# shwetabhardwaj44/EfficientVideoClassification_Youtube8M

Measured on AMD Instinct MI355X. Metric: frames/sec (whole node) H-LSTM teacher+student B=256x300x1152; GAP@20, higher is better.
Workload: dtype bf16; 1 GPU; HierarchicalLstmModel teacher_student every_n=10, lstm_cells=1024x2, MoE(2), batch 256 x 300 x 1152 per GPU; global_batch=256, frames_per_video=300, parallelism=dp1, num_frames=U{120..300}

## Files before the change

### efficientvideoclassification_youtube8m_amd/_lib.py

```python
from __future__ import annotations

import ctypes as C
import os

_HERE = os.path.dirname(os.path.abspath(__file__))
LIB_PATH = os.environ.get("EVC_LIB", os.path.join(_HERE, "libevc_hip.so"))

vp, i32, i64, f32 = C.c_void_p, C.c_int, C.c_int64, C.c_float

SIGNATURES = {
    "evc_check_device": [i32],
    "evc_l2norm_chunk_fwd": [vp, vp, vp, i32, i32, i32, i32, vp, i32, i32, vp, i32, vp, vp, i32, vp, i32, vp, i32, vp],
    "evc_sort_rows_by_len": [vp, i32, i32, vp, vp, vp, vp],
    "evc_frame_counts": [vp, i32, i32, i32, i32, i32, i32, vp, vp, vp, vp],
    "evc_gemm_nt": [vp, i64, vp, i64, vp, i64, i32, i32, i32, vp, i32, i32, vp],
    "evc_gemm_nt_sqnorm": [vp, i64, vp, i64, vp, i64, i32, i32, i32, vp, f32, vp, vp, i64, vp],
    "evc_gemm_tn": [vp, i64, vp, i64, vp, i64, i32, i32, i32, i32, i32, vp],
    "evc_gemm_tn2": [vp, i64, vp, i64, i32, vp, i64, i32, i32, vp, i64, i32, i32, i32, i32, vp],
    "evc_gemm_tn2_rows": [vp, i64, vp, i64, i32, vp, i64, i32, i32, vp, i64, i32, i32, i32, vp, i32, i32, vp],
    "evc_gemm_tn2_slabs": [vp, i64, vp, i64, i32, vp, i64, i32, i32, vp, i64, i64, i32, i32, i32, i32, vp],
    "evc_sum_slabs": [vp, i64, i32, i32, i32, i64, vp, i64, i32, vp],
    "evc_colsum_bf16": [vp, i64, i32, i32, i32, vp, vp],
    "evc_colsum_bf16_det": [vp, i64, i32, i32, i32, vp, vp, i32, vp],
    "evc_lstm_layer_fwd": [vp, vp, vp, vp, i32, i32, i32, i32, i32, vp, vp, vp, vp, i64, vp, vp, vp, vp, vp],
    "evc_lstm_layer_fwd_hp": [vp, vp, i64, vp, i64, vp, vp, i32, i32, i32, i32, vp, vp, vp, vp, vp, i64, vp, vp, vp],
    "evc_gemm_nt_split": [vp, i64, vp, i64, vp, i64, i32, i32, i32, vp, vp],
    "evc_cast_f32_to_f16_wide": [vp, i64, i32, i32, i32, i32, i32, vp, vp],
    "evc_cast_f32_to_bf16_wide": [vp, i64, i32, i32, vp, i64, i32, vp],
    "evc_lstm_layer_fwd_f16": [vp, i64, vp, vp, vp, i32, i32, i32, i32, vp, i32, vp, vp, vp, i64, vp, vp, vp, vp, vp],
    "evc_lstm_layer_fwd_f16_fp8lo": [vp, i64, i32, i64, i32, vp, vp, i32, i32, vp, vp, i32, i32, i32, vp, vp, vp, vp, i64, vp, vp, vp, vp, vp, vp, i32, vp],
    "evc_l2norm_chunk_int": [vp, vp, i32, i32, i32, i32, vp, i32, i32, vp, vp, vp, vp, vp, vp, i32, vp, i32, vp],
    "evc_lstm_level2_fwd_high": [vp, i64, i32, i64, i32, vp, vp, i32, i32, vp, vp, vp, i32, vp, i64, vp, vp, i32, i32, i32, vp, vp, vp, vp, vp, vp, vp, vp, i64,
                                 vp, vp, vp, vp, vp, vp, vp],
    "evc_lstm_layer_fwd_f16_dith": [vp, i64, i32, i64, i32, vp, i64, vp, i64, i32, vp, vp, i32, i32, i32, vp, vp, vp, vp, i64, vp, vp, vp, vp, vp],
    "evc_cast_f32_to_f16_dither": [vp, i64, i32, i64, C.c_uint32, vp, i64, i64, vp],
    "evc_lstm_stack2_fwd_f16_fp8lo": [vp, i32, vp, vp, vp, vp, vp, i32, i32, vp, vp, i32, i32, i32, i32, vp, vp, vp, vp, vp, vp, vp, vp, vp, i64, vp, vp, vp, vp, vp],
    "evc_cast_f32_to_fp8_lo": [vp, i64, i32, i32, i32, i32, i32, vp, i64, vp],
    "evc_cast_f32_to_fp8_lohi": [vp, i64, i32, i32, i32, i32, i32, vp, i64, vp],
    "evc_lstm_layer_bwd": [vp, vp, i32, i32, i32, i32, vp, vp, vp, vp, i64, vp, vp, vp, vp, vp, vp, vp, vp, vp],
    "evc_transpose_to_bf16": [vp, i32, i64, i32, i32, vp, i64, i32, i32, vp],
    "evc_cast_f32_to_bf16": [vp, i64, i32, i32, vp, i64, vp],
    "evc_cast_f32_to_f16": [vp, i64, i32, i32, vp, i64, vp],
    "evc_cast_f32_to_bf16_split": [vp, i64, i32, i32, vp, vp, i64, vp],
# ... 116 lines not shown
```

### efficientvideoclassification_youtube8m_amd/csrc/evc_gemm_tn.hip

```cpp
#include "gemm_shared.h"

struct StoreParamsT {
  float* C; long ldc; int M, N;
  int row_il_H;
  int accumulate, splits, ksteps_per_split;
  long slab_stride;
};

template <class Cfg, bool SEG = false>
__global__ __launch_bounds__(Cfg::NT) void gemm_tn_kernel(GemmOperandsT p, StoreParamsT s, int tiles_m, int tiles_n) {
  const int nwg = tiles_m * tiles_n;
  int bid = blockIdx.x, split = 0;
  if (s.splits > 1) {
    split = bid / nwg;
    bid -= split * nwg;
  }
  const int id = xcd_remap(bid, nwg);
  int tm, tn;
  tile_of(id, tiles_m, tiles_n, tm, tn, s.splits > 1 ? patch_rows(nwg, tiles_n) : 8);
  const int m0 = tm * Cfg::BM;
  int n0 = tn * Cfg::BU;
  int nb = n0;
  if (p.B2) {
    if (n0 >= p.N1) {
      p.B = p.B2; p.ldb = p.ldb2; nb = n0 - p.N1; p.N = s.N - p.N1;
      s.N = p.c_col2 + p.N;
      n0 = p.c_col2 + nb;
    } else {
      p.N = s.N = p.N1;
    }
  }
  if (SEG) {
    int off = split * s.ksteps_per_split, sg = 0;
    p.nk = min(s.ksteps_per_split, p.nk - off);
#pragma unroll
    for (int i = 0; i < 15; ++i) {
      const bool adv = sg == i && i + 1 < p.nseg && off >= (int)p.seg_len[i];
      off -= adv ? (int)p.seg_len[i] : 0;
      sg += adv ? 1 : 0;
    }
    p.seg0 = sg; p.seg_off0 = off;
  } else if (s.splits > 1) {
    const int k0 = split * s.ksteps_per_split;
    p.A += (long)k0 * 32 * p.lda;
    p.B += (long)k0 * 32 * p.ldb;
    p.nk = min(s.ksteps_per_split, p.nk - k0);
  }
  f32x4 acc[Cfg::MI][1][Cfg::NI];
  gemm_mainloop_tn<Cfg, true, TN_LOOP_MODE, SEG>(p, m0, nb, lds_dyn, acc);
  float* C = s.C + split * s.slab_stride;
  const int wave = threadIdx.x >> 6, wc = wave % Cfg::WC;
  const bool plain = s.slab_stride > 0 || (s.splits == 1 && !s.accumulate);
  const bool aligned = (s.ldc % 4) == 0 && ((uintptr_t)C % 16) == 0 && n0 + wc * Cfg::WU + Cfg::WU <= s.N;
  __syncthreads();
  if (plain && aligned) {
    store_tile_via_lds<Cfg, 4, false>(acc, lds_dyn, C, s.ldc, s.M, s.N, m0, n0, nullptr, s.row_il_H);
  } else if (s.splits == 1 && s.accumulate && aligned) {
    store_tile_via_lds<Cfg, 4, false, true>(acc, lds_dyn, C, s.ldc, s.M, s.N, m0, n0, nullptr, s.row_il_H);
  } else if (plain) {
    TileCoordsT<Cfg> tc;
#pragma unroll
    for (int mi = 0; mi < Cfg::MI; ++mi) {
      const int m = m0 + tc.row0 + mi * 16;
      if (m >= s.M) continue;
      const long mo = s.row_il_H > 0 ? (long)(m & 3) * s.row_il_H + (m >> 2) : m;
#pragma unroll
      for (int ni = 0; ni < Cfg::NI; ++ni)
#pragma unroll
        for (int r = 0; r < 4; ++r) {
          const int n = n0 + tc.unit0 + ni * 16 + r;
          if (n < s.N) C[mo * s.ldc + n] = acc[mi][0][ni][r];
        }
    }
  } else {
    store_tile_via_lds<Cfg, 4, true>(acc, lds_dyn, C, s.ldc, s.M, s.N, m0, n0, nullptr, s.row_il_H);
  }
}

static int gemm_tn_impl(const evc_bf16* A, int64_t lda, const evc_bf16* B, int64_t ldb, int N1, const evc_bf16* B2, int64_t ldb2,
                        int c_col2, float* C, int64_t ldc, int M, int N, int K, int row_interleave_H, int accumulate, void* stream,
                        int slab_rows = 0, const int32_t* rows_per_slab = nullptr) {
  EVC_REQUIRE(M >= 8 && N >= 8 && K > 0 && M % 8 == 0 && N % 8 == 0 && K % 32 == 0, EVC_ERR_BAD_SHAPE,
              "evc_gemm_tn: needs M %% 8 == 0, N %% 8 == 0, K %% 32 == 0 (M=%d N=%d K=%d)", M, N, K);
  EVC_REQUIRE(lda % 8 == 0 && ldb % 8 == 0 && ((uintptr_t)A % 16) == 0 && ((uintptr_t)B % 16) == 0, EVC_ERR_BAD_ALIGN,
              "evc_gemm_tn: operands must be 16-byte aligned (lda=%ld ldb=%ld)", (long)lda, (long)ldb);
  EVC_REQUIRE(row_interleave_H == 0 || M == 4 * row_interleave_H, EVC_ERR_BAD_SHAPE, "evc_gemm_tn: row_interleave_H needs M == 4*H");
  EVC_REQUIRE(!B2 || (N1 > 0 && N1 < N && N1 % 256 == 0 && ldb2 % 8 == 0 && ((uintptr_t)B2 % 16) == 0 && c_col2 >= N1), EVC_ERR_BAD_SHAPE,
              "evc_gemm_tn2: N1=%d must be a multiple of 256 inside (0, N=%d), B2 16-byte aligned with ldb2 %% 8 == 0, c_col2=%d >= N1", N1, N, c_col2);
  hipStream_t st = (hipStream_t)stream;
  GemmOperandsT p{A, lda, B, ldb, M, N, K / 32};
  if (B2) { p.B2 = B2; p.ldb2 = ldb2; p.N1 = N1; p.c_col2 = c_col2; }
  bool seg = false;
  if (rows_per_slab && slab_rows > 0 && slab_rows % 32 == 0 && K % slab_rows == 0 && !evc_deterministic()) {
    const int nslabs = K / slab_rows, slab_steps = slab_rows / 32;
    int n = 0, total = 0;
    const long ld_max = lda > ldb ? (long)lda : (long)ldb;
    bool ok = (long)nslabs * slab_steps < 65536 && (long)K * (B2 && ldb2 > ld_max ? (long)ldb2 : ld_max) * 2 < (1L << 32);
    for (int t = 0; t < nslabs && ok; ++t) {
      int r = rows_per_slab[t] < 0 ? 0 : (rows_per_slab[t] > slab_rows ? slab_rows : rows_per_slab[t]);
      const int steps = (r + 31) / 32;
      if (steps == 0) continue;
      if (n == 16) { ok = false; break; }
      p.seg_start[n] = (unsigned short)(t * slab_steps); p.seg_len[n] = (unsigned short)steps;
      ++n; total += steps;
    }
    if (ok && total > 0 && total < K / 32) { seg = true; p.nseg = n; p.nk = total; K = total * 32; }
  }
  typedef TileCfg2<128, 1, 128, 2, 4, 5, true> CfgTn128;
  if (forced_tile() == 11 || (forced_tile() == 0 && K <= 2048 && (long)ceil_div(M, 128) * ceil_div(N, 128) >= 192)) {
    const int tm1 = ceil_div(M, 128), tn1 = ceil_div(N, 128);
    StoreParamsT s1{C, ldc, M, N, row_interleave_H, accumulate, 1, p.nk, 0};
    if (seg) launch_cfg<CfgTn128>(gemm_tn_kernel<CfgTn128, true>, tm1 * tn1, st, p, s1, tm1, tn1);
    else launch_cfg<CfgTn128>(gemm_tn_kernel<CfgTn128>, tm1 * tn1, st, p, s1, tm1, tn1);
    EVC_LAUNCH_CHECK();
    return EVC_OK;
  }
  if (forced_tile() == 0 && N <= 128 && !B2) {
    const int tm1 = ceil_div(M, 128);
    int splits = 256 / tm1;
    if (splits > K / 1024) splits = K / 1024;
    if (splits < 1 || evc_deterministic()) splits = 1;
    while (splits > 1 && (long)ceil_div(p.nk, splits) * (splits - 1) >= p.nk) --splits;
    StoreParamsT s1{C, ldc, M, N, row_interleave_H, accumulate, splits, ceil_div(p.nk, splits), 0};
    if (splits > 1 && !accumulate) EVC_CHECK_HIP(hipMemset2DAsync(C, ldc * sizeof(float), 0, (size_t)N * sizeof(float), M, st));
    if (seg) launch_cfg<CfgTn128>(gemm_tn_kernel<CfgTn128, true>, tm1 * splits, st, p, s1, tm1, 1);
    else launch_cfg<CfgTn128>(gemm_tn_kernel<CfgTn128>, tm1 * splits, st, p, s1, tm1, 1);
    EVC_LAUNCH_CHECK();
    return EVC_OK;
  }
  const int tm = ceil_div(M, CfgPlainV2::BM), tn = ceil_div(N, CfgPlainV2::BU);
  int splits = 256 / (tm * tn);
  if (splits > K / 1024) splits = K / 1024;
  if (splits < 1 || evc_deterministic()) splits = 1;
  StoreParamsT s{C, ldc, M, N, row_interleave_H, accumulate, splits, ceil_div(p.nk, splits), 0};
  if (splits > 1 && !accumulate) EVC_CHECK_HIP(hipMemset2DAsync(C, ldc * sizeof(float), 0, (size_t)N * sizeof(float), M, st));
  if (seg) launch_cfg<CfgPlainV2>(gemm_tn_kernel<CfgPlainV2, true>, tm * tn * splits, st, p, s, tm, tn);
  else launch_cfg<CfgPlainV2>(gemm_tn_kernel<CfgPlainV2>, tm * tn * splits, st, p, s, tm, tn);
  EVC_LAUNCH_CHECK();
  return EVC_OK;
}

extern "C" int evc_gemm_tn2_rows(const evc_bf16* A, int64_t lda, const evc_bf16* B1, int64_t ldb1, int N1, const evc_bf16* B2, int64_t ldb2,
                                 int N2, int c_col2, float* C, int64_t ldc, int M, int slab_rows, int nslabs, const int32_t* rows_per_slab,
                                 int row_interleave_H, int accumulate, void* stream) {
  EVC_REQUIRE(B1 && N1 > 0 && slab_rows > 0 && nslabs > 0 && rows_per_slab && (long)slab_rows * nslabs < (1L << 31), EVC_ERR_BAD_ARG,
              "evc_gemm_tn2_rows: B1, N1, slab_rows, nslabs, rows_per_slab are required");
  EVC_REQUIRE(!B2 || N2 > 0, EVC_ERR_BAD_ARG, "evc_gemm_tn2_rows: N2=%d", N2);
  EVC_REQUIRE(!B2 || accumulate || c_col2 == N1, EVC_ERR_BAD_ARG, "evc_gemm_tn2_rows: segments that are not adjacent in C (c_col2=%d, N1=%d) need accumulate", c_col2, N1);
  return gemm_tn_impl(A, lda, B1, ldb1, B2 ? N1 : 0, B2, ldb2, B2 ? c_col2 : 0, C, ldc, M, N1 + (B2 ? N2 : 0), slab_rows * nslabs, row_interleave_H, accumulate,
                      stream, slab_rows, rows_per_slab);
}

extern "C" int evc_gemm_tn(const evc_bf16* A, int64_t lda, const evc_bf16* B, int64_t ldb, float* C, int64_t ldc,
                           int M, int N, int K, int row_interleave_H, int accumulate, void* stream) {
  return gemm_tn_impl(A, lda, B, ldb, 0, nullptr, 0, 0, C, ldc, M, N, K, row_interleave_H, accumulate, stream);
}

extern "C" int evc_gemm_tn2(const evc_bf16* A, int64_t lda, const evc_bf16* B1, int64_t ldb1, int N1, const evc_bf16* B2, int64_t ldb2,
                            int N2, int c_col2, float* C, int64_t ldc, int M, int K, int row_interleave_H, int accumulate, void* stream) {
  EVC_REQUIRE(B1 && B2 && N1 > 0 && N2 > 0, EVC_ERR_BAD_ARG, "evc_gemm_tn2: two column segments are required");
  EVC_REQUIRE(accumulate || c_col2 == N1, EVC_ERR_BAD_ARG, "evc_gemm_tn2: segments that are not adjacent in C (c_col2=%d, N1=%d) need accumulate "
              "(the split-K join adds into a C the caller has zeroed)", c_col2, N1);
  return gemm_tn_impl(A, lda, B1, ldb1, N1, B2, ldb2, c_col2, C, ldc, M, N1 + N2, K, row_interleave_H, accumulate, stream);
}

extern "C" int evc_gemm_tn_slabs(const evc_bf16* A, int64_t lda, const evc_bf16* B, int64_t ldb, float* slabs, int M, int N, int K,
                                 int nslab, void* stream) {
  EVC_REQUIRE(M >= 8 && N >= 8 && K > 0 && M % 8 == 0 && N % 8 == 0 && K % 32 == 0 && nslab >= 1 && nslab <= K / 32, EVC_ERR_BAD_SHAPE,
              "evc_gemm_tn_slabs: needs M %% 8 == 0, N %% 8 == 0, K %% 32 == 0, 1 <= nslab <= K/32 (M=%d N=%d K=%d nslab=%d)", M, N, K, nslab);
  EVC_REQUIRE(lda % 8 == 0 && ldb % 8 == 0 && ((uintptr_t)A % 16) == 0 && ((uintptr_t)B % 16) == 0, EVC_ERR_BAD_ALIGN,
              "evc_gemm_tn_slabs: operands must be 16-byte aligned (lda=%ld ldb=%ld)", (long)lda, (long)ldb);
  GemmOperandsT p{A, lda, B, ldb, M, N, K / 32};
  const int tm = ceil_div(M, CfgPlainV2::BM), tn = ceil_div(N, CfgPlainV2::BU);
  const int per = ceil_div(p.nk, nslab);
  EVC_REQUIRE((long)per * (nslab - 1) < p.nk, EVC_ERR_BAD_SHAPE, "evc_gemm_tn_slabs: nslab=%d leaves an empty slab at K=%d", nslab, K);
  StoreParamsT s{slabs, N, M, N, 0, 0, nslab, per, (long)M * N};
  launch_cfg<CfgPlainV2>(gemm_tn_kernel<CfgPlainV2>, tm * tn * nslab, (hipStream_t)stream, p, s, tm, tn);
  EVC_LAUNCH_CHECK();
  return EVC_OK;
}

extern "C" int evc_gemm_tn2_slabs(const evc_bf16* A, int64_t lda, const evc_bf16* B1, int64_t ldb1, int N1, const evc_bf16* B2, int64_t ldb2,
                                  int N2, int c_col2, float* slabs, int64_t ldc, int64_t slab_stride, int M, int K, int row_interleave_H,
                                  int nslab, void* stream) {
  const int N = N1 + (B2 ? N2 : 0);
  EVC_REQUIRE(M >= 8 && N1 >= 8 && K > 0 && M % 8 == 0 && N % 8 == 0 && K % 32 == 0 && nslab >= 1 && nslab <= K / 32, EVC_ERR_BAD_SHAPE,
// ... 316 lines not shown
```

### efficientvideoclassification_youtube8m_amd/engine.py

```python
from __future__ import annotations

import math
import os
from collections import OrderedDict

import torch

from . import ops

BF16, F32 = torch.bfloat16, torch.float32


def _align(n, a=16):
    return (n + a - 1) // a * a


def _drain(gen):
    try:
        while True:
            next(gen)
    except StopIteration as e:
        return e.value


# ... 292 lines not shown
            e1.synchronize()
            flops = sum(2.0 * r * 4 * H * (self.kin[l] + (H if t > 0 else 0)) for l in range(2) for t, r in enumerate(rows))
            live = sum(1 for r in rows if r > 0)
            return [(e0.elapsed_time(e1) / reps, live + 1 if live else 0, flops)]
        for l in range(self.L):
            kn, bn = self.names(l)
            gates = self._v(self.gates[l], T, M, H, 2) if self.training else None
            c_all = self._v(self.c_all[l], T + 1, M, H) if self.training else None
            args = (inp, tw.shadow_fwd[kn], tw.store.p(bn), self.lens, T, M, self.kin[l], H, self._hb[l],
                    self.S[:, (2 * l) * H:], self.S[:, (2 * l + 1) * H:], 2 * self.L * H, gates, c_all)
            ops.lstm_layer_fwd(*args, hoist=self.hoist[l], zx_ws=self.zx, plan=plan)
            e0, e1 = torch.cuda.Event(enable_timing=True), torch.cuda.Event(enable_timing=True)
            e0.record()
            for _ in range(reps):
                ops.lstm_layer_fwd(*args, hoist=self.hoist[l], zx_ws=self.zx, plan=plan)
            e1.record()
            e1.synchronize()
            kx = 0 if self.hoist[l] else self.kin[l]
            flops = sum(2.0 * r * 4 * H * (kx + (H if t > 0 else 0)) for t, r in enumerate(rows))
            res.append((e0.elapsed_time(e1) / reps, sum(1 for r in rows if r > 0), flops))
            inp = self._hb[l][1:]
        return res

    def _wgrad_tn(self, dz2, layer_in, h_prev, kin, rows, gW, live=None):
        H = self.H
        n1 = kin // 256 * 256
        if ops.DETERMINISTIC and rows % 32 == 0 and kin % 8 == 0:
            if n1 >= 256 and (kin == n1 or kin - n1 >= 8):
                ops.gemm_tn_det(dz2, layer_in, 4 * H, n1, rows, gW, row_interleave_H=H, accumulate=True, ldc=kin + H, B2=h_prev, N2=H, c_col2=kin)
                if kin > n1:
                    ops.gemm_tn_det(dz2, layer_in[:, n1:], 4 * H, kin - n1, rows, gW[:, n1:kin], row_interleave_H=H, accumulate=True, ldc=kin + H)
            else:
                ops.gemm_tn_det(dz2, layer_in, 4 * H, kin, rows, gW, row_interleave_H=H, accumulate=True, ldc=kin + H)
                ops.gemm_tn_det(dz2, h_prev, 4 * H, H, rows, gW[:, kin:], row_interleave_H=H, accumulate=True, ldc=kin + H)
            return
        if kin == H and kin % 256 == 0:
            ops.gemm_tn2(dz2, layer_in, kin, h_prev, H, 4 * H, rows, gW, row_interleave_H=H, accumulate=True, live_rows=live)
        elif kin - n1 in (64, 128) and n1 >= H and rows >= 16384 and (n1 + H) % 2048 == 0:
            ops.gemm_tn2(dz2, layer_in, n1, h_prev, H, 4 * H, rows, gW, row_interleave_H=H, accumulate=True, c_col2=kin, live_rows=live)
            ops.gemm_tn(dz2, layer_in[:, n1:], 4 * H, kin - n1, rows, gW[:, n1:kin], row_interleave_H=H, lda=dz2.stride(0),
                        ldb=layer_in.stride(0), ldc=kin + H, accumulate=True, live_rows=live)
        else:
            ops.gemm_tn(dz2, layer_in, 4 * H, kin, rows, gW, row_interleave_H=H, ldc=kin + H, accumulate=True, live_rows=live)
            ops.gemm_tn(dz2, h_prev, 4 * H, H, rows, gW[:, kin:], row_interleave_H=H, ldc=kin + H, accumulate=True, live_rows=live)

    def backward(self, dS, need_dx, aux=None, on_layer_grads=None):
        return _drain(self.backward_layers(dS, need_dx, aux, on_layer_grads))

    def backward_layers(self, dS, need_dx, aux=None, on_layer_grads=None):
        tw, H, L, T, plan = self.tw, self.H, self.L, self.T, self.plan
        M = self.Mrun
        assert plan is None or not need_dx, "dX of a row-planned stack would be in slot order"
        dh_above = None
        dx_out = None
        main = torch.cuda.current_stream(tw.device)
        use_tn = (T * M) % 32 == 0 and all(k % 8 == 0 for k in self.kin)
        assert use_tn or not self.use_tn or M == self.M
        fuse_ok = L == 2 and use_tn and not need_dx and M >= 1024 and H % 128 == 0
        small_pair = (L == 2 and self.small_pair and use_tn and M <= 512 and H % 128 == 0 and plan is None and not ops.DETERMINISTIC
                      and self.dc_ws2 is not None)
        if small_pair or (fuse_ok and self.bwd_fuse == "pair"):
            (k0, b0), (k1, b1) = self.names(0), self.names(1)
            dz = [self._v(self.dz[l], T, M, 4 * H) for l in range(2)]
            gb = [tw.store.g(b0), tw.store.g(b1)]
            for g in gb:
                ops.fill_f32(g, 0.0)
            ops.lstm_stack2_bwd(tw.shadow_bwd[k0], tw.shadow_bwd[k1], self.lens, T, M, self.kin[0], H,
                                [self._v(self.gates[l], T, M, H, 2) for l in range(2)],
                                [self._v(self.c_all[l], T + 1, M, H) for l in range(2)], dS,
                                [self._v(self.dc_ws, M, H), self._v(self.dc_ws2, M, H)], dz, gb, plan=plan)
            side = main
            if aux is not None:
                ev = torch.cuda.Event()
                ev.record(main)
                aux.wait_event(ev)
                side = aux
            with torch.cuda.stream(side):
                for l, kn in ((1, k1), (0, k0)):
                    kin = self.kin[l]
                    gW = tw.store.g(kn)
                    dz2 = dz[l].view(T * M, 4 * H)
                    layer_in = (self.x_in if l == 0 else self._hb[0][1:]).reshape(T * M, kin)
                    h_prev = self._hb[l][:T].reshape(T * M, H)
                    ops.fill_f32(gW, 0.0)
                    self._wgrad_tn(dz2, layer_in, h_prev, kin, T * M, gW)
                    if on_layer_grads is not None:
                        on_layer_grads(l)
            if need_dx:
                if self.dx[0] is None:
                    self.dx[0] = torch.empty((T * M, self.kin[0]), dtype=F32, device=tw.device)
                ops.gemm_nt(dz[0].view(T * M, 4 * H), tw.shadow_bwd[k0], T * M, self.kin[0], 4 * H, self.dx[0])
                dx_out = self.dx[0]
            yield 1
            yield 0
            return dx_out
        if fuse_ok and self.bwd_fuse == "fused" and on_layer_grads is not None:
            deferred, user_cb = [], on_layer_grads
            on_layer_grads = deferred.append
        else:
            deferred = user_cb = None
        for l in range(L - 1, -1, -1):
            kn, bn = self.names(l)
            w = tw.shadow_bwd[kn]
            kin = self.kin[l]
            KP = self.KP
            dz = self._v(self.dz[l], T, M, 4 * H)
            gb = tw.store.g(bn)
            det = ops.DETERMINISTIC
# ... 14 lines not shown
            elif l > 0:
                dxl = self._v(self.dx[l], T * M, kin)
                with self._timed("dx_nt", 1, 2.0 * T * M * kin * 4 * H):
                    ops.gemm_nt(dz2, w, T * M, kin, 4 * H, dxl)
                dh_above = dxl
            elif need_dx:
                if self.dx[0] is None:
                    self.dx[0] = torch.empty((T * M, kin), dtype=F32, device=tw.device)
                ops.gemm_nt(dz2, w, T * M, kin, 4 * H, self.dx[0])
                dx_out = self.dx[0]
            side = main
            if aux is not None:
                ev = torch.cuda.Event()
                ev.record(main)
                aux.wait_event(ev)
                side = aux
            with torch.cuda.stream(side):
                gW = tw.store.g(kn)
                layer_in = (self.x_in if l == 0 else self._hb[l - 1][1:]).reshape(T * M, kin)
                h_prev = self._hb[l][:T].reshape(T * M, H)
                if det:
                    ops.colsum_bf16(dz2, T * M, 4 * H, gb, deinterleave_H=H)
                if use_tn:
                    ops.fill_f32(gW, 0.0)
                    with self._timed("wgrad_tn", 1, 2.0 * (sum(rows) if plan is not None else T * M) * 4 * H * (kin + H), stream=side):
                        self._wgrad_tn(dz2, layer_in, h_prev, kin, T * M, gW, live=(rows, M) if plan is not None and M % 32 == 0 else None)
                else:
                    ops.transpose_to_bf16(dz2, T * M, 4 * H, self.dzT, KP, interleave_H=-H)
                    inT = self.xT[:kin]
                    ops.transpose_to_bf16(layer_in, T * M, kin, inT, KP)
                    ops.transpose_to_bf16(h_prev, T * M, H, self.hT_ws, KP)
                    ops.gemm_nt(self.dzT, inT, 4 * H, kin, KP, gW, ldc=kin + H)
                    ops.gemm_nt(self.dzT, self.hT_ws, 4 * H, H, KP, gW[:, kin:], ldc=kin + H)
                if on_layer_grads is not None:
                    on_layer_grads(l)
                if deferred is not None and l == 0:
                    for ll in deferred:
                        user_cb(ll)
            yield l
        return dx_out


class MoeHead:

    GATES, EXPERTS, EBIAS = "classifier/gates/weights", "classifier/experts/weights", "classifier/experts/biases"

    def __init__(self, tower, K, V, Mx):
        self.tw, self.K, self.V, self.Mx = tower, K, V, Mx

# ... 972 lines not shown
```

### efficientvideoclassification_youtube8m_amd/ops.py

```python
from __future__ import annotations

import ctypes as C

import os

import torch

from . import _lib

BF16 = torch.bfloat16
F16 = torch.float16
F32 = torch.float32


def _p(t):
    if t is None:
        return None
    if not t.is_cuda:
        raise _lib.EvcError("evc ops need device tensors (got a CPU tensor); there is no CPU path")
    return t.data_ptr()


def _stream():
    return torch.cuda.current_stream().cuda_stream
# ... 69 lines not shown
    ldc = out.stride(0) if ldc is None else ldc
    ntot = (c_col2 + N2) if B2 is not None else N
    tiles = ((M + 255) // 256) * ((N + N2 + 255) // 256)
    nslab = max(1, min(256 // max(1, tiles), K // 1024))
    while nslab > 1 and ((K // 32 + nslab - 1) // nslab) * (nslab - 1) >= K // 32:
        nslab -= 1
    ws = torch.empty((nslab, M, ntot), dtype=F32, device=out.device)
    _lib.call("evc_gemm_tn2_slabs", _p(A), A.stride(0), _p(B), B.stride(0), N, _p(B2), B2.stride(0) if B2 is not None else 0, N2,
              (c_col2 if c_col2 is not None else N), _p(ws), ntot, M * ntot, M, K, row_interleave_H, nslab, _stream())
    for c0, w in ((0, N),) + (((c_col2, N2),) if B2 is not None else ()):
        _lib.call("evc_sum_slabs", _p(ws[0, :, c0:]), M * ntot, nslab, M, w, ntot, _p(out[:, c0:]), ldc, 1 if accumulate else 0, _stream())
    return out


def gemm_tn2(A, B1, N1, B2, N2, M, K, out, row_interleave_H=0, accumulate=False, ldc=None, c_col2=None, live_rows=None):
    assert A.dtype == BF16 and B1.dtype == BF16 and B2.dtype == BF16 and out.dtype == F32
    if live_rows is not None:
        slab, ns, arr = _slab_rows_arg(live_rows, K)
        _lib.call("evc_gemm_tn2_rows", _p(A), A.stride(0), _p(B1), B1.stride(0), N1, _p(B2), B2.stride(0), N2, N1 if c_col2 is None else c_col2,
                  _p(out), out.stride(0) if ldc is None else ldc, M, slab, ns, arr, row_interleave_H, 1 if accumulate else 0, _stream())
        return out
    _lib.call("evc_gemm_tn2", _p(A), A.stride(0), _p(B1), B1.stride(0), N1, _p(B2), B2.stride(0), N2, N1 if c_col2 is None else c_col2,
              _p(out), out.stride(0) if ldc is None else ldc, M, K, row_interleave_H, 1 if accumulate else 0, _stream())
    return out


def fill_f32(t, value):
    assert t.dtype == F32 and t.is_contiguous()
    _lib.call("evc_fill_f32", _p(t), t.numel(), float(value), _stream())


DETERMINISTIC = os.environ.get("EVC_DETERMINISTIC", "0") not in ("", "0")


def colsum_bf16(x, R, C, out, deinterleave_H=0):
    if DETERMINISTIC and R >= 128:
        ws = torch.empty((128, C), dtype=F32, device=x.device)
        _lib.call("evc_colsum_bf16_det", _p(x), x.stride(0), R, C, deinterleave_H, _p(out), _p(ws), 128, _stream())
        return out
    _lib.call("evc_colsum_bf16", _p(x), x.stride(0), R, C, deinterleave_H, _p(out), _stream())
    return out


def transpose_to_bf16(x, R, C, out, Rpad, ld_in=None, interleave_H=0):
    ld_in = x.stride(0) if ld_in is None else ld_in
    _lib.call("evc_transpose_to_bf16", _p(x), 1 if x.dtype == F32 else 0, ld_in, R, C, _p(out), out.stride(0), Rpad,
# ... 673 lines not shown
```

### include/evc.h

```cpp
#ifndef EVC_H_
#define EVC_H_

#include <stdint.h>

#ifdef __cplusplus
extern "C" {
#endif

#define EVC_OK 0
#define EVC_ERR_BAD_SHAPE (-1)
#define EVC_ERR_BAD_ALIGN (-2)
#define EVC_ERR_UNSUPPORTED_ARCH (-3)
#define EVC_ERR_HIP (-4)
#define EVC_ERR_BAD_ARG (-5)

#define EVC_VERSION 107

typedef uint16_t evc_bf16;
typedef uint16_t evc_f16;

int evc_version(void);
const char* evc_last_error(void);
int evc_check_device(int dev);

// ... 210 lines not shown
int evc_bn_partials_reduce(const float* part, int P, int C, double* ws, void* stream);
int evc_bn_finalize_ema(const double* ws, int R_total, int C, float* mean, float* var, float* moving_mean,
                        float* moving_var, float decay, void* stream);
int evc_dbof_input_bn_apply(const float* r, int B, int S, int F, const float* mean, const float* var, const float* gamma,
                            const float* beta, evc_bf16* r_bn, evc_bf16* r_bn_lo, evc_bf16* xhat, void* stream);
int evc_dbof_cluster_pool_fwd(const evc_bf16* r_bn, const evc_bf16* r_bn_lo, const evc_bf16* wT, const evc_bf16* wT_lo,
                              int B, int S, int F, int C, const float* gamma, evc_bf16* act, float* part, float* xsel,
                              uint8_t* arg, void* stream);
int evc_dbof_input_bn_apply_f16fp8(const float* r, int B, int S, int F, const float* mean, const float* var, const float* gamma,
                                   const float* beta, evc_f16* r_rows, int hi_exp, int lo_exp, evc_bf16* xhat, void* stream);
int evc_dbof_cluster_pool_fwd_f16fp8(const evc_f16* r_rows, const evc_f16* wT16, const uint8_t* wT8, int scale_exp,
                                     int B, int S, int F, int C, const float* gamma, evc_bf16* act, float* part, float* xsel,
                                     uint8_t* arg, void* stream);
int evc_dbof_pool_finish(const float* xsel, int B, int C, const float* mean, const float* var, const float* gamma,
                         const float* beta, float* pooled_f32, evc_bf16* pooled_bf16, evc_bf16* pooled_lo, void* stream);
int evc_dbof_dact(evc_bf16* act, const float* dpooled, const float* pooled, const uint8_t* arg, const float* mean,
                  const float* var, const float* gamma, const double* ws, int R_total, int B, int S, int C, float* dgamma,
                  float* dbeta, void* stream);
int evc_gemm_tn2(const evc_bf16* A, int64_t lda, const evc_bf16* B1, int64_t ldb1, int N1, const evc_bf16* B2, int64_t ldb2,
                 int N2, int c_col2, float* C, int64_t ldc, int M, int K, int row_interleave_H, int accumulate, void* stream);
int evc_gemm_tn2_rows(const evc_bf16* A, int64_t lda, const evc_bf16* B1, int64_t ldb1, int N1, const evc_bf16* B2, int64_t ldb2,
                      int N2, int c_col2, float* C, int64_t ldc, int M, int slab_rows, int nslabs, const int32_t* rows_per_slab,
                      int row_interleave_H, int accumulate, void* stream);
int evc_gemm_tn_slabs(const evc_bf16* A, int64_t lda, const evc_bf16* B, int64_t ldb, float* slabs, int M, int N, int K,
                      int nslab, void* stream);
int evc_gemm_tn2_slabs(const evc_bf16* A, int64_t lda, const evc_bf16* B1, int64_t ldb1, int N1, const evc_bf16* B2, int64_t ldb2,
                       int N2, int c_col2, float* slabs, int64_t ldc, int64_t slab_stride, int M, int K, int row_interleave_H,
                       int nslab, void* stream);
int evc_sum_slabs(const float* slabs, int64_t slab_stride, int nslab, int M, int N, int64_t ld, float* C, int64_t ldc, int accumulate,
                  void* stream);
int evc_dbof_wgrad_finish(const float* slabs, int nslab, int C, int F, const float* W, const float* gamma_in, float* dW,
                          float* dgamma_in, float* dbeta_in, float* part_ws, void* stream);

int evc_netvlad_softmax_fwd(const float* act, int R, int K, const float* mean, const float* var, const float* gamma,
                            const float* beta, float* a, void* stream);
int evc_netvlad_softmax_bwd(const float* a, const float* da, int R, int K, float* dz, void* stream);
int evc_netvlad_aggregate_fwd(const float* a, const float* r, int B, int S, int K, int F, const float* mean, const float* var,
                              const float* gamma, const float* beta, const float* c2, float* V, float* asum, void* stream);
int evc_netvlad_aggregate_bwd(const float* a, const float* r, int B, int S, int K, int F, const float* mean, const float* var,
                              const float* gamma, const float* beta, const float* c2, const float* dV, float* da, float* dx,
                              void* stream);
int evc_netvlad_dcenters(const float* asum, const float* dV, int B, int K, int F, float* dc2, void* stream);
int evc_netvlad_normalize_fwd(const float* V, int B, int K, int F, float* n1, float* n2, float* Y_f32, evc_bf16* Y_bf16,
                              void* stream);
int evc_netvlad_normalize_bwd(const float* V, const float* n1, const float* n2, const float* dY, int B, int K, int F, float* dV,
                              void* stream);
// ... 32 lines not shown
```

Baseline: 7.684 million frames/sec.

## Replace atomic split-K accumulation in LSTM wgrad with last-block join

The split-K weight-gradient GEMM used to zero the output with fill/memset and have every split add its partial into C. Now split 0 writes C directly, the other splits write into a cached per-site workspace, and a per-tile atomic counter lets the last-arriving block sum the partials and store the final tile. This drops the separate zero-fill launches and the contended read-modify-write on C, and the result no longer depends on the order splits finish. The cost is extra workspace memory, a fence and counter round-trip per block, and a serial reduction tail done by one block per tile.

Result: no change. 7.698 million frames/sec, median of 6 (+0.2%).

```diff
diff --git a/efficientvideoclassification_youtube8m_amd/_lib.py b/efficientvideoclassification_youtube8m_amd/_lib.py
--- a/efficientvideoclassification_youtube8m_amd/_lib.py
+++ b/efficientvideoclassification_youtube8m_amd/_lib.py
@@ -19,6 +19,8 @@
     "evc_gemm_tn2": [vp, i64, vp, i64, i32, vp, i64, i32, i32, vp, i64, i32, i32, i32, i32, vp],
     "evc_gemm_tn2_rows": [vp, i64, vp, i64, i32, vp, i64, i32, i32, vp, i64, i32, i32, i32, vp, i32, i32, vp],
     "evc_gemm_tn2_slabs": [vp, i64, vp, i64, i32, vp, i64, i32, i32, vp, i64, i64, i32, i32, i32, i32, vp],
+    "evc_gemm_tn2_join": [vp, i64, vp, i64, i32, vp, i64, i32, i32, vp, i64, i32, i32, i32, vp, i32, vp, i64, vp, i32, vp],
+    "evc_gemm_tn_join_ws": [i32, i32, i32, i32, i32, vp, vp],
     "evc_sum_slabs": [vp, i64, i32, i32, i32, i64, vp, i64, i32, vp],
     "evc_colsum_bf16": [vp, i64, i32, i32, i32, vp, vp],
     "evc_colsum_bf16_det": [vp, i64, i32, i32, i32, vp, vp, i32, vp],
diff --git a/efficientvideoclassification_youtube8m_amd/csrc/evc_gemm_tn.hip b/efficientvideoclassification_youtube8m_amd/csrc/evc_gemm_tn.hip
--- a/efficientvideoclassification_youtube8m_amd/csrc/evc_gemm_tn.hip
+++ b/efficientvideoclassification_youtube8m_amd/csrc/evc_gemm_tn.hip
@@ -5,9 +5,45 @@
   int row_il_H;
   int accumulate, splits, ksteps_per_split;
   long slab_stride;
+  float* join_ws = nullptr; long join_ld = 0, join_stride = 0; unsigned* join_ctr = nullptr;
 };
 
-template <class Cfg, bool SEG = false>
+template <class Cfg>
+__device__ __forceinline__ void join_tile(const StoreParamsT& s, int m0, int n0) {
+  constexpr int Q = Cfg::BU / 4, U = 8;
+  static_assert((Cfg::BM * Q) % (Cfg::NT * U) == 0, "tile must divide into whole batches");
+  const int ncol4 = min(Cfg::BU, s.N - n0) >> 2;
+#pragma unroll 1
+  for (int base = threadIdx.x; base < Cfg::BM * Q; base += Cfg::NT * U) {
+    float4 a[U];
+    long oc[U], ow[U];
+    bool ok[U];
+#pragma unroll
+    for (int u = 0; u < U; ++u) {
+      const int i = base + u * Cfg::NT;
+      const int r = i / Q, c4 = i - r * Q;
+      ok[u] = m0 + r < s.M && c4 < ncol4;
+      const int m = min(m0 + r, s.M - 1), c = n0 + min(c4, ncol4 - 1) * 4;
+      const long orow = s.row_il_H > 0 ? (long)(m & 3) * s.row_il_H + (m >> 2) : m;
+      oc[u] = orow * s.ldc + c;
+      ow[u] = orow * s.join_ld + c;
+      a[u] = *(const float4*)(s.C + oc[u]);
+    }
+    for (int sp = 1; sp < s.splits; ++sp) {
+      const float* w = s.join_ws + (long)(sp - 1) * s.join_stride;
+      float4 v[U];
+#pragma unroll
+      for (int u = 0; u < U; ++u) v[u] = *(const float4*)(w + ow[u]);
+#pragma unroll
+      for (int u = 0; u < U; ++u) { a[u].x += v[u].x; a[u].y += v[u].y; a[u].z += v[u].z; a[u].w += v[u].w; }
+    }
+#pragma unroll
+    for (int u = 0; u < U; ++u)
+      if (ok[u]) *(float4*)(s.C + oc[u]) = a[u];
+  }
+}
+
+template <class Cfg, bool SEG = false, bool JOIN = false>
 __global__ __launch_bounds__(Cfg::NT) void gemm_tn_kernel(GemmOperandsT p, StoreParamsT s, int tiles_m, int tiles_n) {
   const int nwg = tiles_m * tiles_n;
   int bid = blockIdx.x, split = 0;
@@ -48,13 +84,18 @@
   }
   f32x4 acc[Cfg::MI][1][Cfg::NI];
   gemm_mainloop_tn<Cfg, true, TN_LOOP_MODE, SEG>(p, m0, nb, lds_dyn, acc);
+#ifdef EVC_ABLATE_TN_EPI
+  if (s.M > 0) return;
+#endif
   float* C = s.C + split * s.slab_stride;
+  long ldc = s.ldc;
+  if (JOIN && split > 0) { C = s.join_ws + (long)(split - 1) * s.join_stride; ldc = s.join_ld; }
   const int wave = threadIdx.x >> 6, wc = wave % Cfg::WC;
-  const bool plain = s.slab_stride > 0 || (s.splits == 1 && !s.accumulate);
-  const bool aligned = (s.ldc % 4) == 0 && ((uintptr_t)C % 16) == 0 && n0 + wc * Cfg::WU + Cfg::WU <= s.N;
+  const bool plain = JOIN || s.slab_stride > 0 || (s.splits == 1 && !s.accumulate);
+  const bool aligned = (ldc % 4) == 0 && ((uintptr_t)C % 16) == 0 && n0 + wc * Cfg::WU + Cfg::WU <= s.N;
   __syncthreads();
   if (plain && aligned) {
-    store_tile_via_lds<Cfg, 4, false>(acc, lds_dyn, C, s.ldc, s.M, s.N, m0, n0, nullptr, s.row_il_H);
+    store_tile_via_lds<Cfg, 4, false>(acc, lds_dyn, C, ldc, s.M, s.N, m0, n0, nullptr, s.row_il_H);
   } else if (s.splits == 1 && s.accumulate && aligned) {
     store_tile_via_lds<Cfg, 4, false, true>(acc, lds_dyn, C, s.ldc, s.M, s.N, m0, n0, nullptr, s.row_il_H);
   } else if (plain) {
@@ -69,17 +110,60 @@
 #pragma unroll
         for (int r = 0; r < 4; ++r) {
           const int n = n0 + tc.unit0 + ni * 16 + r;
-          if (n < s.N) C[mo * s.ldc + n] = acc[mi][0][ni][r];
+          if (n < s.N) C[mo * ldc + n] = acc[mi][0][ni][r];
         }
     }
   } else {
     store_tile_via_lds<Cfg, 4, true>(acc, lds_dyn, C, s.ldc, s.M, s.N, m0, n0, nullptr, s.row_il_H);
   }
-}
+  if constexpr (JOIN) {
+    asm volatile("s_waitcnt vmcnt(0)" ::: "memory");
+    __syncthreads();
+    unsigned* last_flag = (unsigned*)lds_dyn;
+    if (threadIdx.x == 0) {
+      __builtin_amdgcn_fence(__ATOMIC_RELEASE, "agent");
+      asm volatile("s_waitcnt vmcnt(0)" ::: "memory");
+      const unsigned t = __hip_atomic_fetch_add(s.join_ctr + bid, 1u, __ATOMIC_RELAXED, __HIP_MEMORY_SCOPE_AGENT);
+      const bool last = t == (unsigned)s.splits - 1;
+      if (last) {
+        __hip_atomic_store(s.join_ctr + bid, 0u, __ATOMIC_RELAXED, __HIP_MEMORY_SCOPE_AGENT);
+        __builtin_amdgcn_fence(__ATOMIC_ACQUIRE, "agent");
+        asm volatile("s_waitcnt vmcnt(0)" ::: "memory");
+      }
+      *last_flag = last ? 1u : 0u;
+    }
+    __syncthreads();
+    if (*last_flag == 0u) return;
+    join_tile<Cfg>(s, m0, n0);
+  }
+}
+
+struct TnPlan { int tile, tm, tn, splits; };
+static TnPlan tn_plan(int M, int N, int K, int nk, bool two_seg, bool keep_splits) {
+  if (forced_tile() == 11 || (forced_tile() == 0 && K <= 2048 && (long)ceil_div(M, 128) * ceil_div(N, 128) >= 192))
+    return TnPlan{128, ceil_div(M, 128), ceil_div(N, 128), 1};
+  const bool one = evc_deterministic() && !keep_splits;
+  if (forced_tile() == 0 && N <= 128 && !two_seg) {
+    const int tm1 = ceil_div(M, 128);
+    int splits = 256 / (evc_deterministic() ? ceil_div(M, CfgPlainV2::BM) : tm1);
+    if (splits > K / 1024) splits = K / 1024;
+    if (splits < 1 || one) splits = 1;
+    while (splits > 1 && (long)ceil_div(nk, splits) * (splits - 1) >= nk) --splits;
+    return TnPlan{128, tm1, 1, splits};
+  }
+  const int tm = ceil_div(M, CfgPlainV2::BM), tn = ceil_div(N, CfgPlainV2::BU);
+  int splits = 256 / (tm * tn);
+  if (splits > K / 1024) splits = K / 1024;
+  if (splits < 1 || one) splits = 1;
+  while (splits > 1 && (long)ceil_div(nk, splits) * (splits - 1) >= nk) --splits;
+  return TnPlan{256, tm, tn, splits};
+}
+
+struct TnJoin { float* ws; long ws_floats; unsigned* ctr; int n_ctr; };
 
 static int gemm_tn_impl(const evc_bf16* A, int64_t lda, const evc_bf16* B, int64_t ldb, int N1, const evc_bf16* B2, int64_t ldb2,
                         int c_col2, float* C, int64_t ldc, int M, int N, int K, int row_interleave_H, int accumulate, void* stream,
-                        int slab_rows = 0, const int32_t* rows_per_slab = nullptr) {
+                        int slab_rows = 0, const int32_t* rows_per_slab = nullptr, const TnJoin* jn = nullptr) {
   EVC_REQUIRE(M >= 8 && N >= 8 && K > 0 && M % 8 == 0 && N % 8 == 0 && K % 32 == 0, EVC_ERR_BAD_SHAPE,
               "evc_gemm_tn: needs M %% 8 == 0, N %% 8 == 0, K %% 32 == 0 (M=%d N=%d K=%d)", M, N, K);
   EVC_REQUIRE(lda % 8 == 0 && ldb % 8 == 0 && ((uintptr_t)A % 16) == 0 && ((uintptr_t)B % 16) == 0, EVC_ERR_BAD_ALIGN,
@@ -106,36 +190,32 @@
     }
     if (ok && total > 0 && total < K / 32) { seg = true; p.nseg = n; p.nk = total; K = total * 32; }
   }
-  typedef TileCfg2<128, 1, 128, 2, 4, 5, true> CfgTn128;
-  if (forced_tile() == 11 || (forced_tile() == 0 && K <= 2048 && (long)ceil_div(M, 128) * ceil_div(N, 128) >= 192)) {
-    const int tm1 = ceil_div(M, 128), tn1 = ceil_div(N, 128);
-    StoreParamsT s1{C, ldc, M, N, row_interleave_H, accumulate, 1, p.nk, 0};
-    if (seg) launch_cfg<CfgTn128>(gemm_tn_kernel<CfgTn128, true>, tm1 * tn1, st, p, s1, tm1, tn1);
-    else launch_cfg<CfgTn128>(gemm_tn_kernel<CfgTn128>, tm1 * tn1, st, p, s1, tm1, tn1);
-    EVC_LAUNCH_CHECK();
-    return EVC_OK;
-  }
-  if (forced_tile() == 0 && N <= 128 && !B2) {
-    const int tm1 = ceil_div(M, 128);
-    int splits = 256 / tm1;
-    if (splits > K / 1024) splits = K / 1024;
-    if (splits < 1 || evc_deterministic()) splits = 1;
-    while (splits > 1 && (long)ceil_div(p.nk, splits) * (splits - 1) >= p.nk) --splits;
-    StoreParamsT s1{C, ldc, M, N, row_interleave_H, accumulate, splits, ceil_div(p.nk, splits), 0};
-    if (splits > 1 && !accumulate) EVC_CHECK_HIP(hipMemset2DAsync(C, ldc * sizeof(float), 0, (size_t)N * sizeof(float), M, st));
-    if (seg) launch_cfg<CfgTn128>(gemm_tn_kernel<CfgTn128, true>, tm1 * splits, st, p, s1, tm1, 1);
-    else launch_cfg<CfgTn128>(gemm_tn_kernel<CfgTn128>, tm1 * splits, st, p, s1, tm1, 1);
-    EVC_LAUNCH_CHECK();
-    return EVC_OK;
-  }
-  const int tm = ceil_div(M, CfgPlainV2::BM), tn = ceil_div(N, CfgPlainV2::BU);
-  int splits = 256 / (tm * tn);
-  if (splits > K / 1024) splits = K / 1024;
-  if (splits < 1 || evc_deterministic()) splits = 1;
-  StoreParamsT s{C, ldc, M, N, row_interleave_H, accumulate, splits, ceil_div(p.nk, splits), 0};
-  if (splits > 1 && !accumulate) EVC_CHECK_HIP(hipMemset2DAsync(C, ldc * sizeof(float), 0, (size_t)N * sizeof(float), M, st));
-  if (seg) launch_cfg<CfgPlainV2>(gemm_tn_kernel<CfgPlainV2, true>, tm * tn * splits, st, p, s, tm, tn);
-  else launch_cfg<CfgPlainV2>(gemm_tn_kernel<CfgPlainV2>, tm * tn * splits, st, p, s, tm, tn);
+  const TnPlan pl = tn_plan(M, N, K, p.nk, B2 != nullptr, jn != nullptr);
+  StoreParamsT s{C, ldc, M, N, row_interleave_H, accumulate, pl.splits, ceil_div(p.nk, pl.splits), 0};
+  const bool join = jn && pl.splits > 1;
+  if (join) {
+    const long ld_ws = B2 ? (long)c_col2 + (N - N1) : (long)N;
+    EVC_REQUIRE((long)(pl.splits - 1) * M * ld_ws <= jn->ws_floats && pl.tm * pl.tn <= jn->n_ctr, EVC_ERR_BAD_ARG,
+                "evc_gemm_tn2_join: workspace too small (%d splits of [%d][%ld] need %ld floats, %d counters; see evc_gemm_tn_join_ws)", pl.splits, M, ld_ws,
+                (long)(pl.splits - 1) * M * ld_ws, pl.tm * pl.tn);
+    s.join_ws = jn->ws; s.join_ld = ld_ws; s.join_stride = (long)M * ld_ws; s.join_ctr = jn->ctr;
+  } else if (pl.splits > 1 && !accumulate) {
+    EVC_CHECK_HIP(hipMemset2DAsync(C, ldc * sizeof(float), 0, (size_t)N * sizeof(float), M, st));
+  }
+  const int grid = pl.tm * pl.tn * pl.splits;
+  if (pl.tile == 128) {
+    if (join) {
+      if (seg) launch_cfg<CfgTn128>(gemm_tn_kernel<CfgTn128, true, true>, grid, st, p, s, pl.tm, pl.tn);
+      else launch_cfg<CfgTn128>(gemm_tn_kernel<CfgTn128, false, true>, grid, st, p, s, pl.tm, pl.tn);
+    } else if (seg) launch_cfg<CfgTn128>(gemm_tn_kernel<CfgTn128, true>, grid, st, p, s, pl.tm, pl.tn);
+    else launch_cfg<CfgTn128>(gemm_tn_kernel<CfgTn128>, grid, st, p, s, pl.tm, pl.tn);
+  } else {
+    if (join) {
+      if (seg) launch_cfg<CfgPlainV2>(gemm_tn_kernel<CfgPlainV2, true, true>, grid, st, p, s, pl.tm, pl.tn);
+      else launch_cfg<CfgPlainV2>(gemm_tn_kernel<CfgPlainV2, false, true>, grid, st, p, s, pl.tm, pl.tn);
+    } else if (seg) launch_cfg<CfgPlainV2>(gemm_tn_kernel<CfgPlainV2, true>, grid, st, p, s, pl.tm, pl.tn);
+    else launch_cfg<CfgPlainV2>(gemm_tn_kernel<CfgPlainV2>, grid, st, p, s, pl.tm, pl.tn);
+  }
   EVC_LAUNCH_CHECK();
   return EVC_OK;
 }
@@ -162,6 +242,33 @@
   EVC_REQUIRE(accumulate || c_col2 == N1, EVC_ERR_BAD_ARG, "evc_gemm_tn2: segments that are not adjacent in C (c_col2=%d, N1=%d) need accumulate "
               "(the split-K join adds into a C the caller has zeroed)", c_col2, N1);
   return gemm_tn_impl(A, lda, B1, ldb1, N1, B2, ldb2, c_col2, C, ldc, M, N1 + N2, K, row_interleave_H, accumulate, stream);
+}
+
+extern "C" int evc_gemm_tn2_join(const evc_bf16* A, int64_t lda, const evc_bf16* B1, int64_t ldb1, int N1, const evc_bf16* B2, int64_t ldb2,
+                                 int N2, int c_col2, float* C, int64_t ldc, int M, int K, int slab_rows, const int32_t* rows_per_slab,
+                                 int row_interleave_H, float* ws, int64_t ws_floats, uint32_t* counters, int n_counters, void* stream) {
+  EVC_REQUIRE(B1 && N1 > 0 && C && (!B2 || N2 > 0), EVC_ERR_BAD_ARG, "evc_gemm_tn2_join: B1, N1, C (and N2 with B2) are required");
+  EVC_REQUIRE(ldc % 4 == 0 && ((uintptr_t)C % 16) == 0 && (!B2 || c_col2 % 4 == 0), EVC_ERR_BAD_ALIGN,
+              "evc_gemm_tn2_join: C must be 16-byte aligned with ldc %% 4 == 0 and c_col2 %% 4 == 0 (ldc=%ld c_col2=%d)", (long)ldc, c_col2);
+  EVC_REQUIRE(ws_floats >= 0 && n_counters >= 0 && (ws_floats == 0 || (ws && ((uintptr_t)ws % 16) == 0)) && (n_counters == 0 || counters), EVC_ERR_BAD_ARG,
+              "evc_gemm_tn2_join: workspace (16-byte aligned) / counters");
+  EVC_REQUIRE(!rows_per_slab || (slab_rows > 0 && K % slab_rows == 0), EVC_ERR_BAD_ARG, "evc_gemm_tn2_join: K=%d is not a multiple of slab_rows=%d", K, slab_rows);
+  const TnJoin jn{ws, (long)ws_floats, (unsigned*)counters, n_counters};
+  return gemm_tn_impl(A, lda, B1, ldb1, B2 ? N1 : 0, B2, ldb2, B2 ? c_col2 : 0, C, ldc, M, N1 + (B2 ? N2 : 0), K, row_interleave_H, 0, stream,
+                      rows_per_slab ? slab_rows : 0, rows_per_slab, &jn);
+}
+
+extern "C" int evc_gemm_tn_join_ws(int M, int N1, int N2, int c_col2, int K, int64_t* ws_floats, int32_t* n_counters) {
+  EVC_REQUIRE(M > 0 && N1 > 0 && N2 >= 0 && K > 0 && K % 32 == 0 && ws_floats && n_counters, EVC_ERR_BAD_ARG, "evc_gemm_tn_join_ws: M=%d N1=%d N2=%d K=%d", M, N1, N2, K);
+  const bool strip = forced_tile() == 0 && N1 + N2 <= 128 && N2 == 0;
+  const int tiles = strip ? ceil_div(M, 128) : ceil_div(M, CfgPlainV2::BM) * ceil_div(N1 + N2, CfgPlainV2::BU);
+  int splits = 256 / (strip && evc_deterministic() ? ceil_div(M, CfgPlainV2::BM) : tiles);
+  if (splits > K / 1024) splits = K / 1024;
+  if (splits < 1) splits = 1;
+  const long ld_ws = N2 > 0 ? (long)c_col2 + N2 : (long)N1;
+  *ws_floats = (int64_t)(splits - 1) * M * ld_ws;
+  *n_counters = tiles;
+  return EVC_OK;
 }
 
 extern "C" int evc_gemm_tn_slabs(const evc_bf16* A, int64_t lda, const evc_bf16* B, int64_t ldb, float* slabs, int M, int N, int K,
diff --git a/efficientvideoclassification_youtube8m_amd/engine.py b/efficientvideoclassification_youtube8m_amd/engine.py
--- a/efficientvideoclassification_youtube8m_amd/engine.py
+++ b/efficientvideoclassification_youtube8m_amd/engine.py
@@ -338,27 +338,29 @@
             inp = self._hb[l][1:]
         return res
 
-    def _wgrad_tn(self, dz2, layer_in, h_prev, kin, rows, gW, live=None):
+    def _tn_ws(self, site, M, N1, K, N2=0, c_col2=None):
+        key = (site, torch.cuda.current_stream(self.tw.device).cuda_stream, M, N1, K, N2, c_col2)
+        cache = self.__dict__.setdefault("_tn_join_ws", {})
+        if key not in cache:
+            cache[key] = ops.gemm_tn_join_ws(M, N1, K, N2, c_col2, device=self.tw.device)
+        return cache[key]
+
+    def _wgrad_tn(self, dz2, layer_in, h_prev, kin, rows, gW, live=None, site=0):
         H = self.H
         n1 = kin // 256 * 256
-        if ops.DETERMINISTIC and rows % 32 == 0 and kin % 8 == 0:
-            if n1 >= 256 and (kin == n1 or kin - n1 >= 8):
-                ops.gemm_tn_det(dz2, layer_in, 4 * H, n1, rows, gW, row_interleave_H=H, accumulate=True, ldc=kin + H, B2=h_prev, N2=H, c_col2=kin)
-                if kin > n1:
-                    ops.gemm_tn_det(dz2, layer_in[:, n1:], 4 * H, kin - n1, rows, gW[:, n1:kin], row_interleave_H=H, accumulate=True, ldc=kin + H)
-            else:
-                ops.gemm_tn_det(dz2, layer_in, 4 * H, kin, rows, gW, row_interleave_H=H, accumulate=True, ldc=kin + H)
-                ops.gemm_tn_det(dz2, h_prev, 4 * H, H, rows, gW[:, kin:], row_interleave_H=H, accumulate=True, ldc=kin + H)
-            return
-        if kin == H and kin % 256 == 0:
-            ops.gemm_tn2(dz2, layer_in, kin, h_prev, H, 4 * H, rows, gW, row_interleave_H=H, accumulate=True, live_rows=live)
-        elif kin - n1 in (64, 128) and n1 >= H and rows >= 16384 and (n1 + H) % 2048 == 0:
-            ops.gemm_tn2(dz2, layer_in, n1, h_prev, H, 4 * H, rows, gW, row_interleave_H=H, accumulate=True, c_col2=kin, live_rows=live)
-            ops.gemm_tn(dz2, layer_in[:, n1:], 4 * H, kin - n1, rows, gW[:, n1:kin], row_interleave_H=H, lda=dz2.stride(0),
-                        ldb=layer_in.stride(0), ldc=kin + H, accumulate=True, live_rows=live)
+        M4, ld = 4 * H, kin + H
+        det = ops.DETERMINISTIC
+        if kin % 256 == 0 and (kin == H or (det and kin >= 256)):
+            ops.gemm_tn_join(dz2, layer_in, M4, kin, rows, gW, self._tn_ws((site, 0), M4, kin, rows, H, kin), row_interleave_H=H, ldc=ld,
+                             B2=h_prev, N2=H, c_col2=kin, live_rows=live)
+        elif (kin - n1 in (64, 128) and n1 >= H and rows >= 16384 and (n1 + H) % 2048 == 0) or (det and n1 >= 256 and kin - n1 >= 8):
+            ops.gemm_tn_join(dz2, layer_in, M4, n1, rows, gW, self._tn_ws((site, 0), M4, n1, rows, H, kin), row_interleave_H=H, ldc=ld,
+                             B2=h_prev, N2=H, c_col2=kin, live_rows=live)
+            ops.gemm_tn_join(dz2, layer_in[:, n1:], M4, kin - n1, rows, gW[:, n1:kin], self._tn_ws((site, 1), M4, kin - n1, rows), row_interleave_H=H,
+                             lda=dz2.stride(0), ldb=layer_in.stride(0), ldc=ld, live_rows=live)
         else:
-            ops.gemm_tn(dz2, layer_in, 4 * H, kin, rows, gW, row_interleave_H=H, ldc=kin + H, accumulate=True, live_rows=live)
-            ops.gemm_tn(dz2, h_prev, 4 * H, H, rows, gW[:, kin:], row_interleave_H=H, ldc=kin + H, accumulate=True, live_rows=live)
+            ops.gemm_tn_join(dz2, layer_in, M4, kin, rows, gW, self._tn_ws((site, 0), M4, kin, rows), row_interleave_H=H, ldc=ld, live_rows=live)
+            ops.gemm_tn_join(dz2, h_prev, M4, H, rows, gW[:, kin:], self._tn_ws((site, 1), M4, H, rows), row_interleave_H=H, ldc=ld, live_rows=live)
 
     def backward(self, dS, need_dx, aux=None, on_layer_grads=None):
         return _drain(self.backward_layers(dS, need_dx, aux, on_layer_grads))
@@ -398,8 +400,7 @@
                     dz2 = dz[l].view(T * M, 4 * H)
                     layer_in = (self.x_in if l == 0 else self._hb[0][1:]).reshape(T * M, kin)
                     h_prev = self._hb[l][:T].reshape(T * M, H)
-                    ops.fill_f32(gW, 0.0)
-                    self._wgrad_tn(dz2, layer_in, h_prev, kin, T * M, gW)
+                    self._wgrad_tn(dz2, layer_in, h_prev, kin, T * M, gW, site=l)
                     if on_layer_grads is not None:
                         on_layer_grads(l)
             if need_dx:
@@ -460,9 +461,8 @@
                 if det:
                     ops.colsum_bf16(dz2, T * M, 4 * H, gb, deinterleave_H=H)
                 if use_tn:
-                    ops.fill_f32(gW, 0.0)
                     with self._timed("wgrad_tn", 1, 2.0 * (sum(rows) if plan is not None else T * M) * 4 * H * (kin + H), stream=side):
-                        self._wgrad_tn(dz2, layer_in, h_prev, kin, T * M, gW, live=(rows, M) if plan is not None and M % 32 == 0 else None)
+                        self._wgrad_tn(dz2, layer_in, h_prev, kin, T * M, gW, live=(rows, M) if plan is not None and M % 32 == 0 else None, site=l)
                 else:
                     ops.transpose_to_bf16(dz2, T * M, 4 * H, self.dzT, KP, interleave_H=-H)
                     inT = self.xT[:kin]
diff --git a/efficientvideoclassification_youtube8m_amd/ops.py b/efficientvideoclassification_youtube8m_amd/ops.py
--- a/efficientvideoclassification_youtube8m_amd/ops.py
+++ b/efficientvideoclassification_youtube8m_amd/ops.py
@@ -115,6 +115,25 @@
         return out
     _lib.call("evc_gemm_tn2", _p(A), A.stride(0), _p(B1), B1.stride(0), N1, _p(B2), B2.stride(0), N2, N1 if c_col2 is None else c_col2,
               _p(out), out.stride(0) if ldc is None else ldc, M, K, row_interleave_H, 1 if accumulate else 0, _stream())
+    return out
+
+
+def gemm_tn_join_ws(M, N1, K, N2=0, c_col2=None, device=None):
+    fl, nc = C.c_int64(0), C.c_int32(0)
+    _lib.call("evc_gemm_tn_join_ws", M, N1, N2, (N1 if c_col2 is None else c_col2) if N2 else 0, K, C.byref(fl), C.byref(nc))
+    return (torch.empty(max(4, fl.value), dtype=F32, device=device), torch.zeros(max(1, nc.value), dtype=torch.int32, device=device))
+
+
+def gemm_tn_join(A, B1, M, N1, K, out, ws, row_interleave_H=0, lda=None, ldb=None, ldc=None, B2=None, N2=0, c_col2=None, live_rows=None):
+    assert A.dtype == BF16 and B1.dtype == BF16 and (B2 is None or B2.dtype == BF16) and out.dtype == F32
+    slab, arr = 0, None
+    if live_rows is not None:
+        slab, _, arr = _slab_rows_arg(live_rows, K)
+    img, ctr = ws
+    assert img.dtype == F32 and ctr.dtype == torch.int32
+    _lib.call("evc_gemm_tn2_join", _p(A), A.stride(0) if lda is None else lda, _p(B1), B1.stride(0) if ldb is None else ldb, N1,
+              _p(B2), B2.stride(0) if B2 is not None else 0, N2 if B2 is not None else 0, (N1 if c_col2 is None else c_col2) if B2 is not None else 0,
+              _p(out), out.stride(0) if ldc is None else ldc, M, K, slab, arr, row_interleave_H, _p(img), img.numel(), _p(ctr), ctr.numel(), _stream())
     return out
 
 
diff --git a/include/evc.h b/include/evc.h
--- a/include/evc.h
+++ b/include/evc.h
@@ -256,6 +256,10 @@
 int evc_gemm_tn2_rows(const evc_bf16* A, int64_t lda, const evc_bf16* B1, int64_t ldb1, int N1, const evc_bf16* B2, int64_t ldb2,
                       int N2, int c_col2, float* C, int64_t ldc, int M, int slab_rows, int nslabs, const int32_t* rows_per_slab,
                       int row_interleave_H, int accumulate, void* stream);
+int evc_gemm_tn2_join(const evc_bf16* A, int64_t lda, const evc_bf16* B1, int64_t ldb1, int N1, const evc_bf16* B2, int64_t ldb2,
+                      int N2, int c_col2, float* C, int64_t ldc, int M, int K, int slab_rows, const int32_t* rows_per_slab,
+                      int row_interleave_H, float* ws, int64_t ws_floats, uint32_t* counters, int n_counters, void* stream);
+int evc_gemm_tn_join_ws(int M, int N1, int N2, int c_col2, int K, int64_t* ws_floats, int32_t* n_counters);
 int evc_gemm_tn_slabs(const evc_bf16* A, int64_t lda, const evc_bf16* B, int64_t ldb, float* slabs, int M, int N, int K,
                       int nslab, void* stream);
 int evc_gemm_tn2_slabs(const evc_bf16* A, int64_t lda, const evc_bf16* B1, int64_t ldb1, int N1, const evc_bf16* B2, int64_t ldb2,
```
